# chymaera96/NeuralSampleID

Measured on AMD Instinct MI355X. Metric: audio clips/sec (contrastive step, grafp encoder), higher is better.
Workload: dtype bf16; 1 GPU; B=256 bf16 k=3 hipGraph 2-stream: grafp.yaml GraphEncoder('t') full contrastive step (fwd x2 views + NT-Xent + bwd + clip + Adam), synthetic (64,128) log-mel clip pairs per GPU, random-init weights; global_batch=256, k=3, parallelism=dp1, collectives=none (single process), gemm_arithmetic=bf16 MFMA operands, fp32 accumulate, activation_storage=bf16, views=two HIP streams (parallel graph branches), hipgraph=True

## Files before the change

include/nsid.h:

```cpp
#ifndef NSID_H
#define NSID_H
#include <stddef.h>
#include <stdint.h>

#ifdef __cplusplus
extern "C" {
#endif

#define NSID_OK 0
#define NSID_EINVAL (-1)
#define NSID_ELAUNCH (-2)

#define NSID_ACT_NONE 0
#define NSID_ACT_RELU 1
#define NSID_ACT_LEAKY 2
#define NSID_ACT_ELU 3

#define NSID_ROW_TILE 128

#define NSID_F32 0
#define NSID_BF16 1

#define NSID_GEMM_FP32 0
#define NSID_GEMM_BF16 1
// ... 58 lines not shown
                     float* running_mean, float* running_var, int64_t* num_batches_tracked, float momentum,
                     float eps, float* scale, float* shift, float* mean, float* invstd, void* stream);
int nsid_bn_finalize_deferred(const float* stat, int tiles, int C, int M, const float* gamma, const float* beta, float eps,
                              float* scale, float* shift, float* mean, float* invstd, float* uvar, void* stream);
int nsid_bn_running_update(int n, const int* C, float* const* running_mean, float* const* running_var,
                           int64_t* const* num_batches_tracked, const float* const* mean_a, const float* const* uvar_a,
                           const float* const* mean_b, const float* const* uvar_b, float momentum, void* stream);
int nsid_bn_eval_affine(const float* gamma, const float* beta, const float* running_mean, const float* running_var,
                        float eps, int C, float* scale, float* shift, void* stream);
int nsid_bn_apply(const void* r, const float* scale, const float* shift, int act, const void* residual,
                  void* out, int M, int C, int dtype, void* stream);
int nsid_bn_bwd_reduce(const void* dout, const void* r, int M, int C, const float* scale, const float* shift,
                       const float* mean, const float* invstd, int act, float* partial, int dtype, void* stream);
int nsid_bn_bwd_finalize(const float* partial, int tiles, int C, int M, float* dgamma, float* dbeta, float* coef,
                         void* stream);
int nsid_bn_bwd_finalize_fused(const float* partial, int tiles, int C, int M, float* dgamma, float* dbeta, float* coef,
                               const float* scale, const float* shift, const float* mean, const float* invstd, float* coef4,
                               void* stream);
int nsid_bn_bwd_apply(const void* dout, const void* r, int M, int C, const float* scale, const float* shift,
                      const float* mean, const float* invstd, int act, const float* coef, void* dr, int dtype,
                      void* stream);

int nsid_knn_graph(const void* r, int ldr, const float* scale, const float* shift, int B, int N, int C, int k,
                   int dilation, int32_t* idx, int dtype, void* stream);

int nsid_mr_aggregate_fwd(const void* r, int ldr, const float* scale, const float* shift, const int32_t* idx, int B,
                          int N, int C, int k, void* u, uint8_t* argmax, int dtype, void* stream);
int nsid_mr_aggregate_bwd(const void* du, const int32_t* idx, const uint8_t* argmax, int B, int N, int C, int k,
                          void* dy, int dtype, void* stream);
int nsid_mr_aggregate_bwd_bn(const void* du, const int32_t* idx, const uint8_t* argmax, int B, int N, int C, int k, void* dy,
                             const void* bn_r, int bn_ldr, const float* bn_scale, const float* bn_shift, const float* bn_mean,
                             const float* bn_invstd, int bn_act, float* partial, int dtype, void* stream);

int nsid_batched_index_select_fwd(const float* x, const int32_t* idx, int B, int C, int N, int Nq, int k, float* out,
                                  void* stream);
int nsid_batched_index_select_bwd(const float* dout, const int32_t* idx, int B, int C, int N, int Nq, int k,
                                  float* dx , void* stream);

int nsid_downsample3_fwd(const void* x, int B, int N, int C, const void* wp, int w_dtype, const float* bias, void* out,
                         int Cout, float* stat, int act_dtype, void* stream);
int nsid_downsample3_bwd_weight(const void* dout, const void* x, float* dwp , int B, int N, int C, int Cout,
                                int act_dtype, void* stream);
int nsid_downsample3_bwd_data(const void* dout, const void* wp, const void* w_odd, int w_dtype, void* dx, int B, int N,
                              int C, int Cout, int act_dtype, void* stream);
int nsid_pack_ds_weight_bwd(const float* w, int Cout, int Cin, float* w_odd, void* stream);
int nsid_im2col3_fwd(const void* x, int B, int N, int C, void* col, int dtype, void* stream);
int nsid_im2col3_bwd(const void* dcol, int B, int N, int C, void* dx, int dtype, void* stream);
int nsid_pack_ds_weight(const float* w, int Cout, int Cin, float* wp, void* stream);
int nsid_dsact_fwd(const void* x, int B, int N, int C, const float* in_scale, const float* in_shift, int act_in, const float* w,
                   const float* bias, void* out, int Cout, float* stat, const float* out_scale, const float* out_shift, int act_out,
                   int act_dtype, void* stream);
int nsid_dsact_bwd_weight(const void* dout, const void* x, const float* in_scale, const float* in_shift, int act_in,
                          float* dw , int B, int N, int C, int Cout, int act_dtype, void* stream);
int nsid_dsact_bwd_data(const void* dout, const float* w, void* dx, int B, int N, int C, int Cout, const void* r_prev,
                        const float* scale, const float* shift, const float* mean, const float* invstd, int act, float* partial,
                        int act_dtype, void* stream);
int nsid_dsact_part_rows(int B, int N);
int nsid_ds_prepack(int n, const float* const* w, void* const* wp16, void* const* wb16, float* const* dwp, const int* Cout,
                    const int* Cin, void* stream);
int nsid_unpack_ds_wgrad(const float* dwp, int Cout, int Cin, float* dw , void* stream);

int nsid_peak_patchify_fwd(const float* spec, const float* w, const float* bias, int B, int H, int W, int pb, int pf,
                           int F, void* out, int ldo, float* minmax, int out_dtype, void* stream);
int nsid_peak_patchify_bwd(const float* spec, const float* minmax, const void* out, const void* dout, int ldo,
                           int B, int H, int W, int pb, int pf, int F, float* dw , float* dbias ,
                           int out_dtype, void* stream);
// ... 83 lines not shown
```

neuralsampleid_amd/_lib.py:

```python
import ctypes
import os

import torch

_PKG = os.path.dirname(os.path.abspath(__file__))
LIB_PATH = os.environ.get("NSID_LIB") or os.path.join(_PKG, "libnsid_hip.so")

SIGNATURES = {
    "nsid_set_gemm_precision": "i",
    "nsid_linear_fwd": "pipippiiiiippiipiis",
    "nsid_linear_fwd_res": "pipippipiiiiippiis",
    "nsid_linear_bwd_data": "pipipipiiiiiis",
    "nsid_linear_bwd_data_bn": "pipipipiiiiiipppppips",
    "nsid_linear_bwd_weight": "pipipiiiippiis",
    "nsid_linear_bwd_weight_grouped": "piiis",
    "nsid_colsum_acc": "piiipis",
    "nsid_bn_finalize": "piiipppppffpppps",
    "nsid_bn_finalize_deferred": "piiippfppppps",
    "nsid_bn_running_update": "ippppppppfs",
    "nsid_bn_eval_affine": "ppppfipps",
    "nsid_bn_apply": "pppippiiis",
    "nsid_bn_bwd_reduce": "ppiippppipis",
    "nsid_bn_bwd_finalize": "piiippps",
    "nsid_bn_bwd_apply": "ppiippppippis",
    "nsid_bn_bwd_finalize_fused": "piiipppppppps",
    "nsid_knn_graph": "pippiiiiipis",
    "nsid_mr_aggregate_fwd": "pipppiiiippis",
    "nsid_mr_aggregate_bwd": "pppiiiipis",
    "nsid_im2col3_fwd": "piiipis",
    "nsid_im2col3_bwd": "piiipis",
    "nsid_pack_ds_weight": "piips",
    "nsid_dsact_fwd": "piiippipppipppiis",
    "nsid_dsact_bwd_weight": "ppppipiiiiis",
    "nsid_dsact_bwd_data": "pppiiiipppppipis",
    "nsid_pack_ds_weight_bwd": "piips",
    "nsid_downsample3_fwd": "piiipippipis",
    "nsid_downsample3_bwd_weight": "pppiiiiis",
    "nsid_downsample3_bwd_data": "pppipiiiiis",
    "nsid_unpack_ds_wgrad": "piips",
    "nsid_ds_prepack": "ipppppps",
    "nsid_peak_patchify_fwd": "pppiiiiiipipis",
    "nsid_peak_patchify_bwd": "ppppiiiiiiippis",
    "nsid_peak_patchify_bwd_ws": "ppppiiiiiiipppis",
    "nsid_node_mean_fwd": "piiipis",
    "nsid_node_mean_bwd": "piiipis",
    "nsid_elu_bwd": "pplps",
    "nsid_l2norm_fwd": "piifpps",
    "nsid_l2norm_bwd": "pppiifps",
    "nsid_ntxent_fwd_bwd": "ppiifiipppps",
    "nsid_sumsq_partial": "plps",
    "nsid_adam_step": "pppplpppips",
    "nsid_f32_to_bf16": "ppls",
    "nsid_reflect_pad": "plips",
    "nsid_power_mel_db": "plippiips",
    "nsid_unfold_segments": "piiiiips",
    "nsid_logmel_fft": "pliliippppiplls",
    "nsid_bcn_to_rows": "piiipiis",
    "nsid_rows_to_bcn": "piiiipis",
    "nsid_batched_index_select_fwd": "ppiiiiips",
    "nsid_batched_index_select_bwd": "ppiiiiips",
    "nsid_fill_zero": "pzs",
# ... 137 lines not shown
```

neuralsampleid_amd/csrc/nsid_common.h:

```cpp
#pragma once
#include <hip/hip_runtime.h>
#include <stdint.h>
#include <stdio.h>

#include "../../include/nsid.h"

typedef float f32x2 __attribute__((ext_vector_type(2)));
typedef float f32x4 __attribute__((ext_vector_type(4)));
typedef uint32_t u32x4 __attribute__((ext_vector_type(4)));
typedef __bf16 bf16x4 __attribute__((ext_vector_type(4)));
typedef __bf16 bf16x8 __attribute__((ext_vector_type(8)));

template <typename T> struct Chunk;
template <> struct Chunk<float> {
  static constexpr int N = 4;
  __device__ static __forceinline__ void load(const float* p, float* v) {
    const f32x4 x = *reinterpret_cast<const f32x4*>(p);
#pragma unroll
    for (int e = 0; e < 4; ++e) v[e] = x[e];
  }
  __device__ static __forceinline__ void store(float* p, const float* v) {
    *reinterpret_cast<f32x4*>(p) = f32x4{v[0], v[1], v[2], v[3]};
  }
};
// ... 117 lines not shown
  X(bwd_narrow, -1)                                                                                                           \
  X(g256_min, 512)                                  \
  X(g256_train, 0)                            \
  X(g256_grid, 0)                                           \
  X(wgrad_wide, 1)                                     \
  X(wgrad_rect, 1)                                                                          \
  X(wgrad_wgs_rect, 256)                         \
  X(wgrad_wgs_sq, 1024)                                                                                                       \
  X(wgrad_rect_min, 256)                                                                                                      \
  X(wgrad_sq_min, 256)                                                                                                        \
  X(w3_wgs, 256)                                                                                                              \
  X(w3_min_tiles, 64)                                                                                                         \
  X(knn_strips, 0)                                            \
  X(knn_pair_min, 512)                 \
  X(knn_raw16, 1)               \
  X(knn_raw_wpe, 6)             \
  X(knn_sel_min_n, 128)               \
  X(mr_grid_stride, 0)                              \
  X(mr_split, 0)                                             \
  X(ffn_regs, 3)                \
  X(mr_key_min_k, 8)            \
  X(mr_bwd_sorted_min_k, 3)     \
  X(ffn_waves, 8)                                                \
  X(ffn256, 1)                  \
  X(mrconv_variant, 7)          \
  X(mrconv_pg_wgs, 768)         \
  X(wgg_rows, 4096)             \
  X(wgg_rows_sq, 1024)          \
  X(wgg_rows_gen, 512)          \
  X(bn_fin_tiles, 0)            \
  X(wgg_w3, 1)                  \
  X(wgrad256, 1)                \
  X(wgg_rows256, 4096)          \
  X(ws_gemm, 7)

enum NsidTuneKey {
#define NSID_TUNE_ENUM(name, def) NSID_T_##name,
  NSID_TUNING_TABLE(NSID_TUNE_ENUM)
#undef NSID_TUNE_ENUM
  NSID_T_COUNT
};
extern long g_nsid_tune[NSID_T_COUNT];
static inline long nsid_tune(NsidTuneKey k) { return g_nsid_tune[k]; }

#define NSID_COUNTER_TABLE(X)                                                                  \
  X(gemm_fwd) X(gemm_bwd_data) X(gemm_bwd_weight)              \
  X(gemm_full)                                    \
  X(gemm_ks2)                                                           \
  X(gemm_bwd_split)          \
  X(gemm_split_major)           \
  X(gemm_affine_load)          \
  X(gemm_relu_load)                                                                             \
  X(gemm_bn_sums)              \
  X(gemm_bn_apply_load)     \
  X(gemm256)                                                                   \
  X(ws_fwd) X(ws_bwd_data) X(ws_bwd_bnapply)                    \
  X(wgrad_rect) X(wgrad_square) X(wgrad3) X(wgrad_grouped) X(wgrad_grouped_w3) X(wgrad_grouped_256)                                                 \
  X(bn_bwd_apply) X(bn_bwd_apply_capped)                                                        \
  X(knn2) X(knn2_pair) X(knn2_raw) X(knn_rank) X(knn_sel) X(knn_strips) X(knn_big)                                                  \
  X(mr_fwd_lds) X(mr_fwd_grid) X(mr_fwd_key) X(mr_bwd_sorted)                                                                  \
  X(ffn_fused)                                 \
  X(mrconv_fused)          \
  X(row_sqnorm) X(flat_l2_topk) X(flat_l2_topk_wide) X(seq_scores)    \
  X(clf_node_rows) X(clf_pair_scores)            \
  X(clf_node_rows_n) X(clf_pair_scores_n)        \
  X(clf_mine) X(clf_attn_fwd) X(clf_head_fwd) X(clf_head_bwd) X(clf_attn_bwd) X(clf_seg_reduce)    \
  X(logmel_fft)            \
  X(conv2d_3x3) X(conv2d_1x1) X(ibn_relu) X(stem7_pool) X(gem_pool)

enum NsidCounterKey {
#define NSID_CNT_ENUM(name) NSID_C_##name,
  NSID_COUNTER_TABLE(NSID_CNT_ENUM)
#undef NSID_CNT_ENUM
  NSID_C_COUNT
};
extern long g_nsid_counter[NSID_C_COUNT];
static inline void nsid_count(NsidCounterKey k) { ++g_nsid_counter[k]; }

constexpr int WGG_MAXP = 28;
struct WgProb {
  const void* A[2];
  const void* B[2];
  const float* bsc[2];
  const float* bsh[2];
  float* C;
  int lda, ldb, I, J, R;
  int groups, rchunk;
  int seg_splits, nsplit;
  int tiles, nwg;
  float slope;
  int pad_period, pad_c1;
};
struct WgGroupArgs {
// ... 54 lines not shown
```

neuralsampleid_amd/csrc/wsgemm.hip:

```cpp
#include "nsid_common.h"

namespace {

typedef float f32x16 __attribute__((ext_vector_type(16)));
typedef __attribute__((address_space(3))) void* lds_vptr;
typedef const __attribute__((address_space(1))) void* glb_vptr;
typedef bf16x4 __attribute__((address_space(3)))* lds_bf16x4_ptr;

struct WsArgs {
  const __bf16* x; long ldx;
  const __bf16* w;
  const float* bias;
  const float* in_scale; const float* in_shift; float in_slope;
  __bf16* out; long ldo;
  float* stat; long stat_plane; long stat_ld;
  int M;
};

constexpr int WS_TP = 72;
constexpr int WS_TB = 32 * WS_TP;

template <int CPR>
__device__ __forceinline__ int ws_swz(int j) {
  if constexpr (CPR == 4) return (j >> 2) & 3;
// ... 124 lines not shown
      const bf16x4 v3 = __builtin_amdgcn_ds_read_tr16_b64_v4bf16((lds_bf16x4_ptr)(tr + 4 * WS_TP + 32));
      *reinterpret_cast<bf16x8*>(orow + t * 32) = __builtin_shufflevector(v0, v1, 0, 1, 2, 3, 4, 5, 6, 7);
      *reinterpret_cast<bf16x8*>(orow + 16 * p.ldo + t * 32) = __builtin_shufflevector(v2, v3, 0, 1, 2, 3, 4, 5, 6, 7);
    }

  if constexpr (STAT) {
#pragma unroll
    for (int t = 0; t < GI * NT; ++t) {
      red[((wave * 2 + h) * 2 + 0) * WROWS + t * 32 + j] = ssum[t];
      red[((wave * 2 + h) * 2 + 1) * WROWS + t * 32 + j] = qsum[t];
    }
    __syncthreads();
    for (int c = tid; c < WROWS; c += 256) {
      float s_ = 0.f, q_ = 0.f;
#pragma unroll
      for (int k = 0; k < 8; ++k) { s_ += red[(k * 2 + 0) * WROWS + c]; q_ += red[(k * 2 + 1) * WROWS + c]; }
      const long col = (long)gy * WROWS + c;
      p.stat[(long)tile * p.stat_ld + col] = s_;
      p.stat[p.stat_plane + (long)tile * p.stat_ld + col] = q_;
    }
  }
}

struct WsBwdArgs {
  const __bf16* dy; long ldd;
  const __bf16* w;
  const __bf16* addend; long ldadd;
  __bf16* dx; long ldi;
  const __bf16* bn_r; long bn_ldr;
  const float* bn_scale; const float* bn_shift; const float* bn_mean; const float* bn_invstd; float bn_slope;
  float* bn_partial; long bn_plane; long bn_ld;
  const __bf16* abn_r; const float* abn_coef; long abn_plane; float abn_slope; __bf16* abn_dr; long abn_lddr;
  int M;
};

template <int BPR>
__device__ __forceinline__ int ws_bswz(int row) {
  if constexpr (BPR == 1) return 0;
  else if constexpr (BPR == 2) return (row >> 1) & 1;
  else return row & 3;
}

template <int N, int K, int GI, bool ADD, bool BNR, bool ABN>
__global__ __launch_bounds__(256, (GI * N * K * 2 > 56 * 1024) ? 1 : 2) void ws_bwd_kernel(const WsBwdArgs p) {
  constexpr int KS = N / 16, KT = K / 32;
  constexpr int CPR = K / 8, BPR = K / 32;
  constexpr int WROWS = GI * N, OCH = GI * K;
  constexpr int WBYTES = WROWS * K * 2;
  constexpr int NPIECE = WBYTES / 1024, RPP = 1024 / (2 * K);
  static_assert(N % 16 == 0 && K % 32 == 0 && NPIECE % 4 == 0 && RPP >= 1, "whole fragments, whole pieces per wave");
  constexpr int SIDEB = (ADD || BNR) ? 4 * 2 * 2048 : 0;
  constexpr int REDB = BNR ? 4 * 2 * 2 * OCH * 4 : 0;
  constexpr int COEFB = ABN ? 4 * WROWS * 4 : 0;
  constexpr int LDSB = WBYTES + 4 * WS_TB + SIDEB + REDB + COEFB;
  __shared__ __attribute__((aligned(1024))) char lds[LDSB];
  char* const wimg = lds;
  char* const tb0 = lds + WBYTES;
  char* const side0 = lds + WBYTES + 4 * WS_TB;
  float* const red = reinterpret_cast<float*>(lds + WBYTES + 4 * WS_TB + SIDEB);
  float* const coefs = reinterpret_cast<float*>(lds + WBYTES + 4 * WS_TB + SIDEB + REDB);

  const int tid = threadIdx.x, lane = tid & 63;
  const int wave = __builtin_amdgcn_readfirstlane(tid >> 6);
  const int j = lane & 31, h = lane >> 5;
  const int tile = blockIdx.x, gy = blockIdx.y;
  const long row0 = (long)tile * 128 + wave * 32;

  bf16x8 xf[GI][KS];
  {
    const __bf16* xr = p.dy + (row0 + j) * p.ldd + (long)gy * WROWS + 8 * h;
#pragma unroll
    for (int gi = 0; gi < GI; ++gi)
#pragma unroll
      for (int s = 0; s < KS; ++s) xf[gi][s] = *reinterpret_cast<const bf16x8*>(xr + gi * N + 16 * s);
  }
  bf16x8 rf[ABN ? GI : 1][ABN ? KS : 1];
  if constexpr (ABN) {
    const __bf16* rr = p.abn_r + (row0 + j) * p.ldd + (long)gy * WROWS + 8 * h;
#pragma unroll
    for (int gi = 0; gi < GI; ++gi)
#pragma unroll
      for (int s = 0; s < KS; ++s) rf[gi][s] = *reinterpret_cast<const bf16x8*>(rr + gi * N + 16 * s);
    for (int i = tid; i < WROWS; i += 256) {
#pragma unroll
      for (int v = 0; v < 4; ++v) coefs[v * WROWS + i] = p.abn_coef[v * p.abn_plane + (long)gy * WROWS + i];
    }
  }
  {
    const __bf16* wg = p.w + (long)gy * WROWS * K;
    const int rl = lane / CPR, pc = lane % CPR;
#pragma unroll
    for (int i = 0; i < NPIECE / 4; ++i) {
      const int q = wave * (NPIECE / 4) + i;
      const int row = q * RPP + rl;
      const int lc = (((pc >> 2) ^ ws_bswz<BPR>(row)) << 2) | (pc & 3);
      __builtin_amdgcn_global_load_lds((glb_vptr)(wg + (long)row * K + 8 * lc), (lds_vptr)(wimg + q * 1024), 16, 0, 0);
    }
  }
  const int srow = lane >> 2, scol = 8 * (lane & 3);
  const __bf16* const aptr = ADD ? p.addend + (row0 + srow) * p.ldadd + (long)gy * OCH + scol : nullptr;
  const __bf16* const rptr = BNR ? p.bn_r + (row0 + srow) * p.bn_ldr + (long)gy * OCH + scol : nullptr;
  f32x4 sa[2][2], sr[2][2];
  auto side_load = [&](int t, int par) {
    if constexpr (ADD) {
      sa[par][0] = *reinterpret_cast<const f32x4*>(aptr + t * 32);
      sa[par][1] = *reinterpret_cast<const f32x4*>(aptr + 16 * p.ldadd + t * 32);
    }
    if constexpr (BNR) {
      sr[par][0] = *reinterpret_cast<const f32x4*>(rptr + t * 32);
      sr[par][1] = *reinterpret_cast<const f32x4*>(rptr + 16 * p.bn_ldr + t * 32);
    }
  };
  if constexpr (ADD || BNR) side_load(0, 0);
  wait_vm<0>();
  __syncthreads();

  if constexpr (ABN) {
    const float slope = p.abn_slope;
    const bool masked = slope != 1.f;
    __bf16* const drow = p.abn_dr + (row0 + j) * p.abn_lddr + (long)gy * WROWS + 8 * h;
#pragma unroll
    for (int gi = 0; gi < GI; ++gi)
#pragma unroll
      for (int s = 0; s < KS; ++s) {
        const float* cf = coefs + gi * N + 16 * s + 8 * h;
        const bf16x8 hd = xf[gi][s], hr = rf[gi][s];
        bf16x8 o;
#pragma unroll
        for (int e4 = 0; e4 < 8; e4 += 4) {
          const f32x4 sc = *reinterpret_cast<const f32x4*>(cf + e4), sh = *reinterpret_cast<const f32x4*>(cf + WROWS + e4);
          const f32x4 cp = *reinterpret_cast<const f32x4*>(cf + 2 * WROWS + e4), cq = *reinterpret_cast<const f32x4*>(cf + 3 * WROWS + e4);
#pragma unroll
          for (int e = 0; e < 4; ++e) {
            const float x = (float)hr[e4 + e], d = (float)hd[e4 + e];
            float g = d;
            if (masked) g = (sc[e] * x + sh[e]) > 0.f ? d : d * slope;
            o[e4 + e] = (__bf16)(sc[e] * g + (cp[e] * x + cq[e]));
          }
        }
        xf[gi][s] = o;
        *reinterpret_cast<bf16x8*>(drow + gi * N + 16 * s) = o;
      }
  }

  const int G = lane >> 4, qq = (lane >> 2) & 3, pp = lane & 3;
  const int wq = 8 * h + qq;
  const int wcol = 32 * (G & 1) + 8 * pp;
  char* const tb = tb0 + wave * WS_TB;
  char* const tw = tb + j * WS_TP + 8 * h;
  const char* const tr = tb + (8 * G + qq) * WS_TP + (4 * pp) * 2;
  __bf16* const orow = p.dx + (row0 + (lane & 15)) * p.ldi + (long)gy * OCH + 8 * G;
  char* const simg = side0 + wave * 4096;
  char* const sw_ = simg + lane * 16;
  const char* const sread = simg + (4 * h + qq) * 64 + 32 * (G & 1) + 8 * pp;
  float s0[GI * KT], s1[GI * KT];
#pragma unroll
  for (int t = 0; t < GI * KT; ++t) s0[t] = s1[t] = 0.f;
  const bool bn_unit = p.bn_slope == 1.f;

#pragma unroll
  for (int gi = 0; gi < GI; ++gi)
#pragma unroll
    for (int kt = 0; kt < KT; ++kt) {
      const int t = gi * KT + kt;
      if constexpr (ADD || BNR) {
        if (t + 1 < GI * KT) side_load(t + 1, (t + 1) & 1);
      }
      f32x16 acc;
#pragma unroll
      for (int r = 0; r < 16; ++r) acc[r] = 0.f;
#pragma unroll
      for (int s = 0; s < KS; ++s) {
        const int ra = gi * N + 16 * s + wq, rb = ra + 4;
        const bf16x4 w0 = __builtin_amdgcn_ds_read_tr16_b64_v4bf16(
            (lds_bf16x4_ptr)(wimg + ra * (2 * K) + ((kt ^ ws_bswz<BPR>(ra)) << 6) + wcol));
        const bf16x4 w1 = __builtin_amdgcn_ds_read_tr16_b64_v4bf16(
            (lds_bf16x4_ptr)(wimg + rb * (2 * K) + ((kt ^ ws_bswz<BPR>(rb)) << 6) + wcol));
        acc = __builtin_amdgcn_mfma_f32_32x32x16_bf16(xf[gi][s], __builtin_shufflevector(w0, w1, 0, 1, 2, 3, 4, 5, 6, 7), acc, 0, 0, 0);
      }
      if constexpr (ADD) {
        *reinterpret_cast<f32x4*>(sw_) = sa[t & 1][0];
        *reinterpret_cast<f32x4*>(sw_ + 1024) = sa[t & 1][1];
#pragma unroll
        for (int g = 0; g < 4; ++g) {
          const bf16x4 a4 = __builtin_amdgcn_ds_read_tr16_b64_v4bf16((lds_bf16x4_ptr)(sread + 512 * g));
#pragma unroll
          for (int e = 0; e < 4; ++e) acc[4 * g + e] += (float)a4[e];
        }
      }
      bf16x4 o4[4];
#pragma unroll
      for (int g = 0; g < 4; ++g) {
        o4[g] = __builtin_convertvector((f32x4{acc[4 * g], acc[4 * g + 1], acc[4 * g + 2], acc[4 * g + 3]}), bf16x4);
        *reinterpret_cast<bf16x4*>(tw + 16 * g) = o4[g];
      }
      if constexpr (BNR) {
        *reinterpret_cast<f32x4*>(sw_ + 2048) = sr[t & 1][0];
        *reinterpret_cast<f32x4*>(sw_ + 2048 + 1024) = sr[t & 1][1];
        const long ch = (long)gy * OCH + t * 32 + j;
        const float bsc = p.bn_scale[ch], bsh = p.bn_shift[ch], bmu = p.bn_mean[ch], bis = p.bn_invstd[ch];
        float a0 = 0.f, a1 = 0.f;
#pragma unroll
        for (int g = 0; g < 4; ++g) {
          const bf16x4 r4 = __builtin_amdgcn_ds_read_tr16_b64_v4bf16((lds_bf16x4_ptr)(sread + 2048 + 512 * g));
#pragma unroll
          for (int e = 0; e < 4; ++e) {
            const float dyv = (float)o4[g][e], xx = (float)r4[e];
            float gg = dyv;
            if (!bn_unit) gg = (bsc * xx + bsh) > 0.f ? dyv : dyv * p.bn_slope;
            a0 += gg;
            a1 += gg * ((xx - bmu) * bis);
          }
        }
        s0[t] = a0; s1[t] = a1;
      }
      const bf16x4 v0 = __builtin_amdgcn_ds_read_tr16_b64_v4bf16((lds_bf16x4_ptr)(tr));
      const bf16x4 v1 = __builtin_amdgcn_ds_read_tr16_b64_v4bf16((lds_bf16x4_ptr)(tr + 4 * WS_TP));
      const bf16x4 v2 = __builtin_amdgcn_ds_read_tr16_b64_v4bf16((lds_bf16x4_ptr)(tr + 32));
      const bf16x4 v3 = __builtin_amdgcn_ds_read_tr16_b64_v4bf16((lds_bf16x4_ptr)(tr + 4 * WS_TP + 32));
      *reinterpret_cast<bf16x8*>(orow + t * 32) = __builtin_shufflevector(v0, v1, 0, 1, 2, 3, 4, 5, 6, 7);
      *reinterpret_cast<bf16x8*>(orow + 16 * p.ldi + t * 32) = __builtin_shufflevector(v2, v3, 0, 1, 2, 3, 4, 5, 6, 7);
    }

  if constexpr (BNR) {
#pragma unroll
    for (int t = 0; t < GI * KT; ++t) {
      red[((wave * 2 + h) * 2 + 0) * OCH + t * 32 + j] = s0[t];
      red[((wave * 2 + h) * 2 + 1) * OCH + t * 32 + j] = s1[t];
    }
    __syncthreads();
    for (int c = tid; c < OCH; c += 256) {
      float a0 = 0.f, a1 = 0.f;
#pragma unroll
      for (int k = 0; k < 8; ++k) { a0 += red[(k * 2 + 0) * OCH + c]; a1 += red[(k * 2 + 1) * OCH + c]; }
      const long col = (long)gy * OCH + c;
      p.bn_partial[(long)tile * p.bn_ld + col] = a0;
      p.bn_partial[p.bn_plane + (long)tile * p.bn_ld + col] = a1;
    }
  }
}

template <int N, int K, int GI>
int ws_bwd_launch_t(const WsBwdArgs& p, int gy, hipStream_t s) {
  const dim3 grid(p.M / 128, gy), block(256);
  const bool add = p.addend != nullptr, bnr = p.bn_r != nullptr;
#define WS_BWD_GO(ABN_)                                                                                   \
  do {                                                                                                    \
    if (add) {                                                                                            \
      if (bnr) NSID_LAUNCH((ws_bwd_kernel<N, K, GI, true, true, ABN_>), grid, block, 0, s, p);             \
      else NSID_LAUNCH((ws_bwd_kernel<N, K, GI, true, false, ABN_>), grid, block, 0, s, p);                \
    } else {                                                                                              \
      if (bnr) NSID_LAUNCH((ws_bwd_kernel<N, K, GI, false, true, ABN_>), grid, block, 0, s, p);            \
      else NSID_LAUNCH((ws_bwd_kernel<N, K, GI, false, false, ABN_>), grid, block, 0, s, p);               \
    }                                                                                                     \
  } while (0)
  if (p.abn_r != nullptr) WS_BWD_GO(true);
  else WS_BWD_GO(false);
#undef WS_BWD_GO
  return nsid_launch_status();
}

template <int K, int NOUT, int GI>
int ws_launch(const WsArgs& p, int gy, bool aff, bool stat, hipStream_t s) {
  const dim3 grid(p.M / 128, gy), block(256);
  if (aff) {
    if constexpr (GI > 1) return 1;
    else {
      if (stat) NSID_LAUNCH((ws_fwd_kernel<K, NOUT, GI, true, true>), grid, block, 0, s, p);
      else NSID_LAUNCH((ws_fwd_kernel<K, NOUT, GI, true, false>), grid, block, 0, s, p);
    }
  } else {
    if (stat) NSID_LAUNCH((ws_fwd_kernel<K, NOUT, GI, false, true>), grid, block, 0, s, p);
    else NSID_LAUNCH((ws_fwd_kernel<K, NOUT, GI, false, false>), grid, block, 0, s, p);
  }
  return nsid_launch_status();
}

}

__attribute__((visibility("hidden")))
int nsid_ws_fwd_launch(const void* x, int ldx, const void* w, const float* bias, void* out, int ldo, int M, int Nout, int K,
                       int groups, const float* in_scale, const float* in_shift, float in_slope, float* stat, long stat_plane,
                       long stat_ld, hipStream_t stream) {
  if (M % 128 != 0 || ldx % 8 != 0 || ldo % 8 != 0 || ldx < groups * K || ldo < groups * Nout) return 1;
  if (!nsid_aligned16(x) || !nsid_aligned16(w) || !nsid_aligned16(out)) return 1;
  if ((in_scale != nullptr) != (in_shift != nullptr)) return 1;
  if (in_scale && (!nsid_aligned16(in_scale) || !nsid_aligned16(in_shift))) return 1;
  WsArgs p{};
  p.x = static_cast<const __bf16*>(x); p.ldx = ldx;
  p.w = static_cast<const __bf16*>(w);
  p.bias = bias;
// ... 25 lines not shown
                            const void* abn_r, const float* abn_coef, long abn_plane, float abn_slope, void* abn_dr, long abn_lddr,
                            hipStream_t stream) {
  if (abn_r && (!abn_coef || !abn_dr || ldd != groups * Nout || abn_lddr % 8 != 0 || !nsid_aligned16(abn_r) || !nsid_aligned16(abn_dr) ||
                !nsid_aligned16(abn_coef) || abn_plane % 4 != 0)) return 1;
  if (M % 128 != 0 || ldd % 8 != 0 || ldi % 8 != 0 || ldd < groups * Nout || ldi < groups * K) return 1;
  if (!nsid_aligned16(dout) || !nsid_aligned16(w) || !nsid_aligned16(din)) return 1;
  if (addend && (ldadd % 8 != 0 || ldadd < groups * K || !nsid_aligned16(addend))) return 1;
  if (bn_r && (bn_ldr % 8 != 0 || !nsid_aligned16(bn_r) || !bn_scale || !bn_shift || !bn_mean || !bn_invstd || !bn_partial)) return 1;
  WsBwdArgs p{};
  p.dy = static_cast<const __bf16*>(dout); p.ldd = ldd;
  p.w = static_cast<const __bf16*>(w);
  p.addend = static_cast<const __bf16*>(addend); p.ldadd = ldadd;
  p.dx = static_cast<__bf16*>(din); p.ldi = ldi;
  p.bn_r = static_cast<const __bf16*>(bn_r); p.bn_ldr = bn_ldr;
  p.bn_scale = bn_scale; p.bn_shift = bn_shift; p.bn_mean = bn_mean; p.bn_invstd = bn_invstd; p.bn_slope = bn_slope;
  p.bn_partial = bn_partial; p.bn_plane = bn_plane; p.bn_ld = bn_ld;
  p.abn_r = static_cast<const __bf16*>(abn_r); p.abn_coef = abn_coef; p.abn_plane = abn_plane; p.abn_slope = abn_slope;
  p.abn_dr = static_cast<__bf16*>(abn_dr); p.abn_lddr = abn_lddr;
  p.M = M;
#define WS_CASE(N_, K_, G_, GI_)                                                   \
  if (Nout == N_ && K == K_ && groups == G_) return ws_bwd_launch_t<N_, K_, GI_>(p, G_ / GI_, stream)
  WS_CASE(64, 64, 1, 1);
  WS_CASE(32, 32, 4, 4);
  WS_CASE(64, 128, 1, 1);
  WS_CASE(256, 64, 1, 1);
  WS_CASE(64, 256, 1, 1);
  WS_CASE(128, 128, 1, 1);
  WS_CASE(64, 64, 4, 4);
  WS_CASE(128, 256, 1, 1);
  WS_CASE(128, 128, 4, 1);
#undef WS_CASE
  return 1;
}
```

neuralsampleid_amd/functional.py:

```python
from typing import Dict, List, Optional

import torch

from . import ops
from .ops import ACT_ELU, ACT_LEAKY, ACT_NONE, ACT_RELU, BNAffine

Tensor = torch.Tensor


class KnnTape:

    def __init__(self, replay: Optional[List[Tensor]] = None, cyclic: bool = False, patch=None):
        self.replay = list(replay) if replay is not None else None
        self.recorded: List[Tensor] = []
        self.pos = 0
        self.cyclic = cyclic
        self.patch = list(patch) if patch is not None else None
        self.patched: List[Tensor] = []


TAPE: Optional[KnnTape] = None

EXACT_BIAS_GRAD = False

# ... 296 lines not shown
    if fold_eval(training, S) and a1 is not None and a1.identity:
        gg, gb, grm, grv, _, _ = _bn(P, S, pre + "1.")
        wgf, bgf = ops.folded_conv_bn(ops.w2d(P[pre + "0.weight"]), P[pre + "0.bias"], gg, gb, grm, grv)
        r2, a2 = ops.mrconv_fused_fwd(r1, idx, B, N, C, wgf, bgf), None
    if r2 is None:
        u, amax = ops.mr_aggregate_fwd(r1, idx, B, N, C, a1, want_argmax=S is not None)
        r2, a2 = conv_bn(u, M, C // 2, C // 2, P[pre + "0.weight"], P[pre + "0.bias"], _bn(P, S, pre + "1."), training,
                         groups=4, folded_act=ACT_RELU)
    if fold_eval(training, S):
        return conv_bn(r2, M, 2 * C, C, P["fc2.0.weight"], P["fc2.0.bias"], _bn(P, S, "fc2.1."), training,
                       in_aff=a2, act_in=ACT_RELU, residual=x0)[0]
    r3, a3 = conv_bn(r2, M, 2 * C, C, P["fc2.0.weight"], P["fc2.0.bias"], _bn(P, S, "fc2.1."), training,
                     in_aff=a2, act_in=ACT_RELU)
    x1 = ops.bn_apply(r3, a3, ACT_NONE, residual=x0)
    if S is not None:
        S.update(x0=x0, r1=r1, a1=a1, idx=idx, amax=amax, u=u, r2=r2, a2=a2, r3=r3, a3=a3, B=B, N=N)
        if CHAIN is not None:
            CHAIN.consume(S)
            CHAIN.produce(S, r3, a3, ACT_NONE)
    return x1


def grapher_backward(dx1: Tensor, P, S, G) -> Tensor:
    x0, r1, a1, idx, amax, u, r2, a2, r3, a3 = (S[k_] for k_ in ("x0", "r1", "a1", "idx", "amax", "u", "r2", "a2",
                                                                  "r3", "a3"))
    B, N = S["B"], S["N"]
    M, C = x0.shape
    pre = "graph_conv.gconv.nn."
    dr3, dv, part2 = ops.bn_backward_linear_bwd_data(dx1, r3, a3, ACT_NONE, G["fc2.1.weight"], G["fc2.1.bias"], _link_partial(S),
                                                     ops.w2d(P["fc2.0.weight"]), M, C, 2 * C, 1, bn=(r2, a2, ACT_RELU),
                                                     site=ops.SITE_FC2, inplace=False)
    _bias_grad_before_bn(dr3, G["fc2.0.bias"])
    _wgrad(dr3, r2, ops.w2d(G["fc2.0.weight"]), M, C, 2 * C, 1, a2.scale, a2.shift, ACT_RELU)
    dr2, du, _ = ops.bn_backward_linear_bwd_data(dv, r2, a2, ACT_RELU, G[pre + "1.weight"], G[pre + "1.bias"], part2,
                                                 ops.w2d(P[pre + "0.weight"]), M, C // 2, C // 2, 4, site=ops.SITE_GCONV)
    _bias_grad_before_bn(dr2, G[pre + "0.bias"])
    _wgrad(dr2, u, ops.w2d(G[pre + "0.weight"]), M, C // 2, C // 2, 4)
    dy, part1 = ops.mr_aggregate_bwd(du, idx, amax, B, N, C, bn=(r1, a1, ACT_NONE))
    dr1, dx0, part = ops.bn_backward_linear_bwd_data(dy, r1, a1, ACT_NONE, G["fc1.1.weight"], G["fc1.1.bias"], part1,
                                                     ops.w2d(P["fc1.0.weight"]), M, C, C, 1, addend=dx1, bn=_link_in(S) or False,
                                                     site=ops.SITE_FC1)
    _bias_grad_before_bn(dr1, G["fc1.0.bias"])
    _wgrad(dr1, x0, ops.w2d(G["fc1.0.weight"]), M, C, C)
    _store_partial(S, part)
    return dx0


def ffn_forward(x1: Tensor, P, S: Optional[dict], training: bool) -> Tensor:
    M, C = x1.shape
    H = P["fc1.0.weight"].shape[0]
    if fold_eval(training, S) and C in (64, 128, 256) and H == 4 * C and M % (256 if C == 256 else 128) == 0:
        g1, be1, rm1, rv1, _, _ = _bn(P, S, "fc1.1.")
        g2, be2, rm2, rv2, _, _ = _bn(P, S, "fc2.1.")
        w1f, b1f = ops.folded_conv_bn(ops.w2d(P["fc1.0.weight"]), None, g1, be1, rm1, rv1)
        w2f, b2f = ops.folded_conv_bn(ops.w2d(P["fc2.0.weight"]), None, g2, be2, rm2, rv2)
        out = ops.ffn_fused_fwd(x1, w1f, b1f, w2f, b2f, M, C, H)
        if out is not None:
            return out
    r4, a4 = conv_bn(x1, M, C, H, P["fc1.0.weight"], None, _bn(P, S, "fc1.1."), training, folded_act=ACT_RELU)
    if fold_eval(training, S):
        return conv_bn(r4, M, H, C, P["fc2.0.weight"], None, _bn(P, S, "fc2.1."), training, in_aff=a4, act_in=ACT_RELU,
                       residual=x1)[0]
    r5, a5 = conv_bn(r4, M, H, C, P["fc2.0.weight"], None, _bn(P, S, "fc2.1."), training, in_aff=a4, act_in=ACT_RELU)
    x2 = ops.bn_apply(r5, a5, ACT_NONE, residual=x1)
    if S is not None:
        S.update(x1=x1, r4=r4, a4=a4, r5=r5, a5=a5)
        if CHAIN is not None:
            CHAIN.consume(S)
            CHAIN.produce(S, r5, a5, ACT_NONE)
    return x2

# ... 295 lines not shown
```

neuralsampleid_amd/ops.py:

```python
import os
from typing import Optional, Tuple

import torch

from ._lib import call, get_tuning, launch_counters, lib, reset_tuning, set_tuning

ACT_NONE, ACT_RELU, ACT_LEAKY, ACT_ELU = 0, 1, 2, 3
ROW_TILE = 128
BN_MOMENTUM = 0.1
BN_EPS = 1e-5


class KernelProfile:

    def __init__(self):
        self.records = []
        self.bracket_ms = self._empty_bracket_ms()

    @staticmethod
    def plug(ms: float = 120.0) -> None:
        torch.cuda._sleep(int(ms * 1e-3 * 2.0e9))

    @staticmethod
    def _empty_bracket_ms(n: int = 64) -> float:
# ... 688 lines not shown
def mr_bwd_sums_fused(du, N, C, k) -> bool:
    kmin = get_tuning("mr_bwd_sorted_min_k")
    return bool(FUSE_MR_BWD_SUMS and du.dtype == torch.bfloat16 and kmin > 0 and k >= kmin and N * C == 16384 and C & (C - 1) == 0
                and 64 <= C <= 512)


FUSE_MR_BWD_SUMS = True


def mr_aggregate_bwd(du, idx, amax, B, N, C, bn=None):
    dt = _act(du)
    k = idx.shape[-1]
    dy = torch.empty((B * N, C), device=du.device, dtype=du.dtype)
    nbytes = float(B) * N * (3 * C * du.element_size() + k * 4 + C)
    if bn is not None and mr_bwd_sums_fused(du, N, C, k):
        r, aff, act = bn
        _chk(aff.scale, aff.shift, aff.mean, aff.invstd)
        partial = torch.empty((2, B, C), device=du.device, dtype=torch.float32)
        rc = [0]

        def launch():
            rc[0] = lib.nsid_mr_aggregate_bwd_bn(_p(du), _p(idx), _p(amax), B, N, C, k, _p(dy), _p(r), r.shape[-1], _p(aff.scale),
                                                 _p(aff.shift), _p(aff.mean), _p(aff.invstd), act, _p(partial), dt, _stream())
        _timed("mr_bwd_sorted_kernel +bn_sums", 0.0, nbytes + float(B) * N * C * r.element_size(), launch, (B * N, C, 2 * C, 1))
        if rc[0] == 0:
            return dy, partial
        if PROFILE is not None:
            PROFILE.records.pop()
    c0 = _cnt("mr_bwd_sorted")
    _timed(lambda: "mr_bwd_sorted_kernel" if _cnt("mr_bwd_sorted") > c0 else "mr_bwd_kernel", 0.0, nbytes, lambda: call(
        "nsid_mr_aggregate_bwd", _p(du), _p(idx), _p(amax), B, N, C, k, _p(dy), dt, _stream()),
        (B * N, C, 2 * C, 1))
    return (dy, None) if bn is not None else dy


def ds_out_nodes(N: int) -> int:
    return (N - 1) // 2 + 1


def im2col3_fwd(x, B, N, C) -> torch.Tensor:
    dt = _act(x)
    col = torch.empty((B * ds_out_nodes(N), 3 * C), device=x.device, dtype=x.dtype)
    call("nsid_im2col3_fwd", _p(x), B, N, C, _p(col), dt, _stream())
    return col


def im2col3_bwd(dcol, B, N, C) -> torch.Tensor:
    dt = _act(dcol)
    dx = torch.empty((B * N, C), device=dcol.device, dtype=dcol.dtype)
    call("nsid_im2col3_bwd", _p(dcol), B, N, C, _p(dx), dt, _stream())
    return dx


class DsPrep:

    def __init__(self):
        self.entries = {}

    MAX_LAYERS = 8

    def purge(self) -> None:
        for ptr in [k for k, e in self.entries.items() if e["wref"]() is None or e["wref"]().data_ptr() != k]:
            del self.entries[ptr]

    def register(self, w) -> None:
        import weakref
# ... 711 lines not shown
```

Baseline: 35930 clips/s.

## Fuse grouped-conv backward data with max-relative aggregation backward and BN sums

Adds a templated AGG variant of the ws_bwd_kernel that keeps the grouped-conv input gradient in LDS instead of writing it out. Inside the same tile it builds a per-node CSR of neighbour sources and scatters the max-relative aggregation backward using the argmax indices. It then accumulates the downstream BN backward partial sums before writing. This removes the separate mr_aggregate_bwd launch and the du round trip through global memory. In exchange it adds LDS pressure, per-tile atomics and serial neighbour loops, and it only works when each 128-row tile holds whole clips (N divides 128), with a fallback path otherwise.

After: 36250 clips/s, median of 6. Within noise of the previous version (+0.9%).

```diff
diff --git a/include/nsid.h b/include/nsid.h
--- a/include/nsid.h
+++ b/include/nsid.h
@@ -114,6 +114,13 @@
                              const void* bn_r, int bn_ldr, const float* bn_scale, const float* bn_shift, const float* bn_mean,
                              const float* bn_invstd, int bn_act, float* partial, int dtype, void* stream);
 
+int nsid_gconv_bwd_aggr(const void* dy, const void* r, const float* coef4, int act, void* dr, const void* w, int w_dtype,
+                        const void* addend, int ldadd, void* din, int ldi, int M, int Nout, int K, int groups, int act_dtype,
+                        const void* bn_r, const float* bn_scale, const float* bn_shift, const float* bn_mean, const float* bn_invstd,
+                        int bn_act, float* bn_partial, const int32_t* idx, const uint8_t* argmax, int B, int N, int k, void* agg_dy,
+                        const void* agg_r, int agg_ldr, const float* agg_scale, const float* agg_shift, const float* agg_mean,
+                        const float* agg_invstd, int agg_act, float* agg_partial, void* stream);
+
 int nsid_batched_index_select_fwd(const float* x, const int32_t* idx, int B, int C, int N, int Nq, int k, float* out,
                                   void* stream);
 int nsid_batched_index_select_bwd(const float* dout, const int32_t* idx, int B, int C, int N, int Nq, int k,
diff --git a/neuralsampleid_amd/_lib.py b/neuralsampleid_amd/_lib.py
--- a/neuralsampleid_amd/_lib.py
+++ b/neuralsampleid_amd/_lib.py
@@ -27,6 +27,7 @@
     "nsid_knn_graph": "pippiiiiipis",
     "nsid_mr_aggregate_fwd": "pipppiiiippis",
     "nsid_mr_aggregate_bwd": "pppiiiipis",
+    "nsid_gconv_bwd_aggr": "pppippipipiiiiiipppppip" + "ppiii" + "ppippppip" + "s",
     "nsid_im2col3_fwd": "piiipis",
     "nsid_im2col3_bwd": "piiipis",
     "nsid_pack_ds_weight": "piips",
diff --git a/neuralsampleid_amd/csrc/nsid_common.h b/neuralsampleid_amd/csrc/nsid_common.h
--- a/neuralsampleid_amd/csrc/nsid_common.h
+++ b/neuralsampleid_amd/csrc/nsid_common.h
@@ -173,7 +173,9 @@
   X(wgg_w3, 1)                  \
   X(wgrad256, 1)                \
   X(wgg_rows256, 4096)          \
-  X(ws_gemm, 7)
+  X(ws_gemm, 7)                 \
+  X(gconv_bwd_aggr, 1)          \
+  X(gconv_bwd_aggr_max_k, 8)
 
 enum NsidTuneKey {
 #define NSID_TUNE_ENUM(name, def) NSID_T_##name,
@@ -199,7 +201,7 @@
   X(wgrad_rect) X(wgrad_square) X(wgrad3) X(wgrad_grouped) X(wgrad_grouped_w3) X(wgrad_grouped_256)                                                 \
   X(bn_bwd_apply) X(bn_bwd_apply_capped)                                                        \
   X(knn2) X(knn2_pair) X(knn2_raw) X(knn_rank) X(knn_sel) X(knn_strips) X(knn_big)                                                  \
-  X(mr_fwd_lds) X(mr_fwd_grid) X(mr_fwd_key) X(mr_bwd_sorted)                                                                  \
+  X(mr_fwd_lds) X(mr_fwd_grid) X(mr_fwd_key) X(mr_bwd_sorted) X(gconv_bwd_aggr)                                                             \
   X(ffn_fused)                                 \
   X(mrconv_fused)          \
   X(row_sqnorm) X(flat_l2_topk) X(flat_l2_topk_wide) X(seq_scores)    \
diff --git a/neuralsampleid_amd/csrc/wsgemm.hip b/neuralsampleid_amd/csrc/wsgemm.hip
--- a/neuralsampleid_amd/csrc/wsgemm.hip
+++ b/neuralsampleid_amd/csrc/wsgemm.hip
@@ -180,7 +180,13 @@
   float* bn_partial; long bn_plane; long bn_ld;
   const __bf16* abn_r; const float* abn_coef; long abn_plane; float abn_slope; __bf16* abn_dr; long abn_lddr;
   int M;
+  const int32_t* ag_idx; const uint8_t* ag_amax; __bf16* ag_dy; int ag_N; int ag_k; int ag_C;
+  const __bf16* ag_r; long ag_ldr;
+  const float* ag_scale; const float* ag_shift; const float* ag_mean; const float* ag_invstd; float ag_slope;
+  float* ag_partial; long ag_plane;
 };
+
+constexpr int WS_AG_KMAX = 32;
 
 template <int BPR>
 __device__ __forceinline__ int ws_bswz(int row) {
@@ -189,7 +195,7 @@
   else return row & 3;
 }
 
-template <int N, int K, int GI, bool ADD, bool BNR, bool ABN>
+template <int N, int K, int GI, bool ADD, bool BNR, bool ABN, bool AGG = false>
 __global__ __launch_bounds__(256, (GI * N * K * 2 > 56 * 1024) ? 1 : 2) void ws_bwd_kernel(const WsBwdArgs p) {
   constexpr int KS = N / 16, KT = K / 32;
   constexpr int CPR = K / 8, BPR = K / 32;
@@ -200,8 +206,18 @@
   constexpr int SIDEB = (ADD || BNR) ? 4 * 2 * 2048 : 0;
   constexpr int REDB = BNR ? 4 * 2 * 2 * OCH * 4 : 0;
   constexpr int COEFB = ABN ? 4 * WROWS * 4 : 0;
-  constexpr int LDSB = WBYTES + 4 * WS_TB + SIDEB + REDB + COEFB;
+  static_assert(!AGG || (ABN && !ADD && !BNR), "the aggregation form exists for the grouped-conv site only");
+  constexpr int CH = OCH / 2;
+  constexpr int AG_OS = 2 * CH + 8, AG_AS = CH + 4;
+  constexpr int AG0 = WBYTES + 4 * WS_TB + SIDEB + REDB + COEFB;
+  constexpr int AGB = AGG ? 128 * AG_AS + 128 * 4 + 132 * 4 + 128 * WS_AG_KMAX * 2 : 0;
+  constexpr int LDSB = AG0 + AGB;
+  static_assert(!AGG || (128 * AG_OS <= WBYTES + 4 * WS_TB && LDSB <= 80 * 1024 && AG0 % 16 == 0), "two workgroups per CU");
   __shared__ __attribute__((aligned(1024))) char lds[LDSB];
+  char* const ag_am = lds + AG0;
+  int* const ag_cnt = reinterpret_cast<int*>(lds + AG0 + 128 * AG_AS);
+  int* const ag_start = ag_cnt + 128;
+  uint16_t* const ag_src = reinterpret_cast<uint16_t*>(ag_start + 132);
   char* const wimg = lds;
   char* const tb0 = lds + WBYTES;
   char* const side0 = lds + WBYTES + 4 * WS_TB;
@@ -243,6 +259,40 @@
       const int row = q * RPP + rl;
       const int lc = (((pc >> 2) ^ ws_bswz<BPR>(row)) << 2) | (pc & 3);
       __builtin_amdgcn_global_load_lds((glb_vptr)(wg + (long)row * K + 8 * lc), (lds_vptr)(wimg + q * 1024), 16, 0, 0);
+    }
+  }
+  if constexpr (AGG) {
+    const int k = p.ag_k, E = 128 * k, cn = p.ag_N;
+    const int32_t* const nbb = p.ag_idx + (long)tile * 128 * k;
+    if (tid < 128) ag_cnt[tid] = 0;
+    const uint8_t* const amb = p.ag_amax + (long)tile * 128 * p.ag_C + gy * CH;
+    for (int q = tid; q < 128 * (CH / 16); q += 256) {
+      const int row = q / (CH / 16), c16 = q % (CH / 16);
+      const u32x4 a = *reinterpret_cast<const u32x4*>(amb + (long)row * p.ag_C + 16 * c16);
+      uint32_t* const d = reinterpret_cast<uint32_t*>(ag_am + row * AG_AS + 16 * c16);
+      d[0] = a[0]; d[1] = a[1]; d[2] = a[2]; d[3] = a[3];
+    }
+    __syncthreads();
+    for (int e = tid; e < E; e += 256) {
+      const int m = e / k;
+      atomicAdd(&ag_cnt[(m / cn) * cn + min(max(nbb[e], 0), cn - 1)], 1);
+    }
+    __syncthreads();
+    if (tid < 64) {
+      const int c0 = ag_cnt[2 * tid], c1 = ag_cnt[2 * tid + 1];
+      int inc = c0 + c1;
+#pragma unroll
+      for (int o2 = 1; o2 < 64; o2 <<= 1) { const int v = __shfl_up(inc, o2, 64); if (tid >= o2) inc += v; }
+      const int run = inc - c0 - c1;
+      ag_start[2 * tid] = run; ag_cnt[2 * tid] = run;
+      ag_start[2 * tid + 1] = run + c0; ag_cnt[2 * tid + 1] = run + c0;
+      if (tid == 63) ag_start[128] = inc;
+    }
+    __syncthreads();
+    for (int e = tid; e < E; e += 256) {
+      const int m = e / k;
+      const int pos = atomicAdd(&ag_cnt[(m / cn) * cn + min(max(nbb[e], 0), cn - 1)], 1);
+      ag_src[pos] = (uint16_t)((m << 8) | (e - m * k));
     }
   }
   const int srow = lane >> 2, scol = 8 * (lane & 3);
@@ -304,6 +354,7 @@
   float s0[GI * KT], s1[GI * KT];
 #pragma unroll
   for (int t = 0; t < GI * KT; ++t) s0[t] = s1[t] = 0.f;
+  u32x4 du8[AGG ? 2 : 1][AGG ? GI * KT : 1];
   const bool bn_unit = p.bn_slope == 1.f;
 
 #pragma unroll
@@ -366,9 +417,95 @@
       const bf16x4 v1 = __builtin_amdgcn_ds_read_tr16_b64_v4bf16((lds_bf16x4_ptr)(tr + 4 * WS_TP));
       const bf16x4 v2 = __builtin_amdgcn_ds_read_tr16_b64_v4bf16((lds_bf16x4_ptr)(tr + 32));
       const bf16x4 v3 = __builtin_amdgcn_ds_read_tr16_b64_v4bf16((lds_bf16x4_ptr)(tr + 4 * WS_TP + 32));
-      *reinterpret_cast<bf16x8*>(orow + t * 32) = __builtin_shufflevector(v0, v1, 0, 1, 2, 3, 4, 5, 6, 7);
-      *reinterpret_cast<bf16x8*>(orow + 16 * p.ldi + t * 32) = __builtin_shufflevector(v2, v3, 0, 1, 2, 3, 4, 5, 6, 7);
-    }
+      if constexpr (AGG) {
+        du8[0][t] = __builtin_bit_cast(u32x4, __builtin_shufflevector(v0, v1, 0, 1, 2, 3, 4, 5, 6, 7));
+        du8[1][t] = __builtin_bit_cast(u32x4, __builtin_shufflevector(v2, v3, 0, 1, 2, 3, 4, 5, 6, 7));
+      } else {
+        *reinterpret_cast<bf16x8*>(orow + t * 32) = __builtin_shufflevector(v0, v1, 0, 1, 2, 3, 4, 5, 6, 7);
+        *reinterpret_cast<bf16x8*>(orow + 16 * p.ldi + t * 32) = __builtin_shufflevector(v2, v3, 0, 1, 2, 3, 4, 5, 6, 7);
+      }
+    }
+
+  if constexpr (AGG) {
+    constexpr int T = GI * KT;
+    char* const odd = lds;
+    const int rl = wave * 32 + (lane & 15);
+    __syncthreads();
+    float own[2][T][4];
+#pragma unroll
+    for (int rr = 0; rr < 2; ++rr)
+#pragma unroll
+      for (int t = 0; t < T; ++t) {
+        const u32x4 w4 = du8[rr][t];
+        *reinterpret_cast<uint2*>(odd + (rl + 16 * rr) * AG_OS + 2 * (16 * t + 4 * G)) =
+            uint2{(w4[0] >> 16) | (w4[1] & 0xffff0000u), (w4[2] >> 16) | (w4[3] & 0xffff0000u)};
+#pragma unroll
+        for (int e = 0; e < 4; ++e) own[rr][t][e] = __uint_as_float(w4[e] << 16) - __uint_as_float(w4[e] & 0xffff0000u);
+      }
+    __syncthreads();
+#pragma unroll
+    for (int rr = 0; rr < 2; ++rr) {
+      const int p1 = ag_start[rl + 16 * rr + 1];
+      for (int q = ag_start[rl + 16 * rr]; q < p1; ++q) {
+        const uint32_t s2 = ag_src[q];
+        const uint32_t m = s2 >> 8, jj = s2 & 255u;
+        const char* const ob = odd + m * AG_OS + 8 * G;
+        const char* const ab = ag_am + m * AG_AS + 4 * G;
+#pragma unroll
+        for (int t = 0; t < T; ++t) {
+          const uint2 o = *reinterpret_cast<const uint2*>(ob + 32 * t);
+          const uint32_t a = *reinterpret_cast<const uint32_t*>(ab + 16 * t);
+          own[rr][t][0] += (a & 255u) == jj ? __uint_as_float(o.x << 16) : 0.f;
+          own[rr][t][1] += ((a >> 8) & 255u) == jj ? __uint_as_float(o.x & 0xffff0000u) : 0.f;
+          own[rr][t][2] += ((a >> 16) & 255u) == jj ? __uint_as_float(o.y << 16) : 0.f;
+          own[rr][t][3] += (a >> 24) == jj ? __uint_as_float(o.y & 0xffff0000u) : 0.f;
+        }
+      }
+    }
+    __syncthreads();
+    float* const red = reinterpret_cast<float*>(lds);
+    const bool masked = p.ag_slope != 1.f;
+    const long grow = (long)tile * 128 + rl;
+#pragma unroll
+    for (int t = 0; t < T; ++t) {
+      const int cl = 16 * t + 4 * G;
+      const long ch = (long)gy * CH + cl;
+      const f32x4 bmu = *reinterpret_cast<const f32x4*>(p.ag_mean + ch), bis = *reinterpret_cast<const f32x4*>(p.ag_invstd + ch);
+      f32x4 bsc = {1.f, 1.f, 1.f, 1.f}, bsh = {0.f, 0.f, 0.f, 0.f};
+      if (masked) { bsc = *reinterpret_cast<const f32x4*>(p.ag_scale + ch); bsh = *reinterpret_cast<const f32x4*>(p.ag_shift + ch); }
+      float a0[4] = {0.f, 0.f, 0.f, 0.f}, a1[4] = {0.f, 0.f, 0.f, 0.f};
+#pragma unroll
+      for (int rr = 0; rr < 2; ++rr) {
+        const bf16x4 o4 = __builtin_convertvector((f32x4{own[rr][t][0], own[rr][t][1], own[rr][t][2], own[rr][t][3]}), bf16x4);
+        *reinterpret_cast<bf16x4*>(p.ag_dy + (grow + 16 * rr) * p.ag_C + ch) = o4;
+        const bf16x4 x4 = *reinterpret_cast<const bf16x4*>(p.ag_r + (grow + 16 * rr) * p.ag_ldr + ch);
+#pragma unroll
+        for (int e = 0; e < 4; ++e) {
+          const float dyv = (float)o4[e], xx = (float)x4[e];
+          float gg = dyv;
+          if (masked) gg = (bsc[e] * xx + bsh[e]) > 0.f ? dyv : dyv * p.ag_slope;
+          a0[e] += gg;
+          a1[e] += gg * ((xx - bmu[e]) * bis[e]);
+        }
+      }
+#pragma unroll
+      for (int o2 = 1; o2 < 16; o2 <<= 1)
+#pragma unroll
+        for (int e = 0; e < 4; ++e) { a0[e] += __shfl_xor(a0[e], o2, 64); a1[e] += __shfl_xor(a1[e], o2, 64); }
+      if ((lane & 15) == 0) {
+        *reinterpret_cast<f32x4*>(red + (wave * 2 + 0) * CH + cl) = f32x4{a0[0], a0[1], a0[2], a0[3]};
+        *reinterpret_cast<f32x4*>(red + (wave * 2 + 1) * CH + cl) = f32x4{a1[0], a1[1], a1[2], a1[3]};
+      }
+    }
+    __syncthreads();
+    const int cpt = 128 / p.ag_N, wpc = 4 / cpt;
+    for (int i = tid; i < cpt * 2 * CH; i += 256) {
+      const int clip = i / (2 * CH), which = (i / CH) & 1, c = i % CH;
+      float a = 0.f;
+      for (int w2 = 0; w2 < wpc; ++w2) a += red[((clip * wpc + w2) * 2 + which) * CH + c];
+      p.ag_partial[which * p.ag_plane + ((long)tile * cpt + clip) * p.ag_C + gy * CH + c] = a;
+    }
+  }
 
   if constexpr (BNR) {
 #pragma unroll
@@ -405,6 +542,12 @@
   if (p.abn_r != nullptr) WS_BWD_GO(true);
   else WS_BWD_GO(false);
 #undef WS_BWD_GO
+  return nsid_launch_status();
+}
+
+template <int N, int K, int GI>
+int ws_bwd_aggr_launch_t(const WsBwdArgs& p, int gy, hipStream_t s) {
+  NSID_LAUNCH((ws_bwd_kernel<N, K, GI, false, false, true, true>), dim3(p.M / 128, gy), dim3(256), 0, s, p);
   return nsid_launch_status();
 }
 
@@ -496,3 +639,44 @@
 #undef WS_CASE
   return 1;
 }
+
+extern "C" int nsid_gconv_bwd_aggr(const void* dy, const void* r, const float* coef4, int act, void* dr, const void* w, int w_dtype,
+                                   const void* addend, int ldadd, void* din, int ldi, int M, int Nout, int K, int groups, int act_dtype,
+                                   const void* bn_r, const float* bn_scale, const float* bn_shift, const float* bn_mean,
+                                   const float* bn_invstd, int bn_act, float* bn_partial, const int32_t* idx, const uint8_t* argmax, int B,
+                                   int N, int k, void* agg_dy, const void* agg_r, int agg_ldr, const float* agg_scale,
+                                   const float* agg_shift, const float* agg_mean, const float* agg_invstd, int agg_act, float* agg_partial,
+                                   void* stream) {
+  (void)ldadd; (void)din; (void)ldi; (void)bn_scale; (void)bn_shift; (void)bn_mean; (void)bn_invstd; (void)bn_act; (void)bn_partial;
+  NSID_REQUIRE(dy && r && coef4 && dr && w && idx && argmax && agg_dy && agg_r && agg_scale && agg_shift && agg_mean && agg_invstd &&
+               agg_partial && M > 0 && Nout > 0 && K > 0 && groups > 0 && B > 0 && N > 0 && k > 0 && k <= 255);
+  NSID_REQUIRE(NSID_DTYPE_OK(act_dtype) && NSID_DTYPE_OK(w_dtype) && (long)B * N == (long)M && dr != dy && dr != r);
+  NSID_REQUIRE(act == NSID_ACT_NONE || act == NSID_ACT_RELU || act == NSID_ACT_LEAKY);
+  NSID_REQUIRE(agg_act == NSID_ACT_NONE || agg_act == NSID_ACT_RELU || agg_act == NSID_ACT_LEAKY);
+  if (nsid_tune(NSID_T_gconv_bwd_aggr) == 0 || act_dtype != NSID_BF16 || w_dtype != NSID_BF16 || addend != nullptr || bn_r != nullptr)
+    return 1;
+  if (N > 128 || 128 % N != 0 || M % 128 != 0 || k > WS_AG_KMAX || k > nsid_tune(NSID_T_gconv_bwd_aggr_max_k) || groups != 4 || Nout != K)
+    return 1;
+  if (!((K == 64 && N == 128) || (K == 128 && N == 64))) return 1;
+  const int C = groups * K / 2;
+  NSID_REQUIRE(agg_ldr % 8 == 0 && agg_ldr >= C && nsid_aligned16(dy) && nsid_aligned16(r) && nsid_aligned16(coef4) && nsid_aligned16(dr) &&
+               nsid_aligned16(w) && nsid_aligned16(argmax) && nsid_aligned16(agg_dy) && nsid_aligned16(agg_r) && nsid_aligned16(agg_scale) &&
+               nsid_aligned16(agg_shift) && nsid_aligned16(agg_mean) && nsid_aligned16(agg_invstd));
+  auto slope_of = [](int a) { return a == NSID_ACT_RELU ? 0.f : (a == NSID_ACT_LEAKY ? 0.2f : 1.f); };
+  WsBwdArgs p{};
+  p.dy = static_cast<const __bf16*>(dy); p.ldd = (long)groups * Nout;
+  p.w = static_cast<const __bf16*>(w);
+  p.ldi = (long)groups * K;
+  p.abn_r = static_cast<const __bf16*>(r); p.abn_coef = coef4; p.abn_plane = (long)groups * Nout; p.abn_slope = slope_of(act);
+  p.abn_dr = static_cast<__bf16*>(dr); p.abn_lddr = (long)groups * Nout;
+  p.bn_slope = 1.f;
+  p.M = M;
+  p.ag_idx = idx; p.ag_amax = argmax; p.ag_dy = static_cast<__bf16*>(agg_dy); p.ag_N = N; p.ag_k = k; p.ag_C = C;
+  p.ag_r = static_cast<const __bf16*>(agg_r); p.ag_ldr = agg_ldr;
+  p.ag_scale = agg_scale; p.ag_shift = agg_shift; p.ag_mean = agg_mean; p.ag_invstd = agg_invstd; p.ag_slope = slope_of(agg_act);
+  p.ag_partial = agg_partial; p.ag_plane = (long)B * C;
+  nsid_count(NSID_C_gconv_bwd_aggr);
+  hipStream_t s = static_cast<hipStream_t>(stream);
+  if (K == 64) return ws_bwd_aggr_launch_t<64, 64, 4>(p, 1, s);
+  return ws_bwd_aggr_launch_t<128, 128, 1>(p, 4, s);
+}
diff --git a/neuralsampleid_amd/functional.py b/neuralsampleid_amd/functional.py
--- a/neuralsampleid_amd/functional.py
+++ b/neuralsampleid_amd/functional.py
@@ -352,11 +352,17 @@
                                                      site=ops.SITE_FC2, inplace=False)
     _bias_grad_before_bn(dr3, G["fc2.0.bias"])
     _wgrad(dr3, r2, ops.w2d(G["fc2.0.weight"]), M, C, 2 * C, 1, a2.scale, a2.shift, ACT_RELU)
-    dr2, du, _ = ops.bn_backward_linear_bwd_data(dv, r2, a2, ACT_RELU, G[pre + "1.weight"], G[pre + "1.bias"], part2,
-                                                 ops.w2d(P[pre + "0.weight"]), M, C // 2, C // 2, 4, site=ops.SITE_GCONV)
+    fused = ops.gconv_bwd_aggregate(dv, r2, a2, ACT_RELU, G[pre + "1.weight"], G[pre + "1.bias"], part2, ops.w2d(P[pre + "0.weight"]),
+                                    M, C // 2, C // 2, 4, idx, amax, B, N, C, bn=(r1, a1, ACT_NONE))
+    if fused is not None:
+        dr2, dy, part1 = fused
+    else:
+        dr2, du, _ = ops.bn_backward_linear_bwd_data(dv, r2, a2, ACT_RELU, G[pre + "1.weight"], G[pre + "1.bias"], part2,
+                                                     ops.w2d(P[pre + "0.weight"]), M, C // 2, C // 2, 4, site=ops.SITE_GCONV)
     _bias_grad_before_bn(dr2, G[pre + "0.bias"])
     _wgrad(dr2, u, ops.w2d(G[pre + "0.weight"]), M, C // 2, C // 2, 4)
-    dy, part1 = ops.mr_aggregate_bwd(du, idx, amax, B, N, C, bn=(r1, a1, ACT_NONE))
+    if fused is None:
+        dy, part1 = ops.mr_aggregate_bwd(du, idx, amax, B, N, C, bn=(r1, a1, ACT_NONE))
     dr1, dx0, part = ops.bn_backward_linear_bwd_data(dy, r1, a1, ACT_NONE, G["fc1.1.weight"], G["fc1.1.bias"], part1,
                                                      ops.w2d(P["fc1.0.weight"]), M, C, C, 1, addend=dx1, bn=_link_in(S) or False,
                                                      site=ops.SITE_FC1)
diff --git a/neuralsampleid_amd/ops.py b/neuralsampleid_amd/ops.py
--- a/neuralsampleid_amd/ops.py
+++ b/neuralsampleid_amd/ops.py
@@ -744,6 +744,55 @@
         "nsid_mr_aggregate_bwd", _p(du), _p(idx), _p(amax), B, N, C, k, _p(dy), dt, _stream()),
         (B * N, C, 2 * C, 1))
     return (dy, None) if bn is not None else dy
+
+
+FUSE_GCONV_BWD_AGGR = 1
+
+
+def gconv_bwd_aggregate(dv, r2, a2: "BNAffine", act, dgamma, dbeta, partial, w, M, Nout, K, groups, idx, amax, B, N, C, bn):
+    k = idx.shape[-1]
+    if not (FUSE_GCONV_BWD_AGGR and partial is not None and dv.dtype == torch.bfloat16 and r2.dtype == torch.bfloat16 and
+            M == B * N and M % 128 == 0 and groups == 4 and Nout == K and (K, N) in ((64, 128), (128, 64)) and 2 * C == groups * K and
+            k <= min(32, get_tuning("gconv_bwd_aggr_max_k")) and tuple(r2.shape) == (M, groups * Nout) and tuple(dv.shape) == (M, groups * Nout) and
+            get_tuning("gconv_bwd_aggr") != 0):
+        return None
+    dt = _act(dv, r2)
+    wop, wdt = _weight(w, dt, K)
+    r1, a1, act1 = bn
+    if wdt != BF16 or r1.dtype != torch.bfloat16 or tuple(r1.shape) != (M, C):
+        return None
+    _chk(a1.scale, a1.shift, a1.mean, a1.invstd)
+    s = _stream()
+    ptiles = partial.shape[1]
+    CC = groups * Nout
+    coef = torch.empty((6, CC), device=r2.device, dtype=torch.float32)
+    if not (DIAG_SKIP_FINALIZE & 2):
+        _tk("bn_bwd_finalize_kernel", 8.0 * ptiles * CC + 40.0 * CC, lambda: call(
+            "nsid_bn_bwd_finalize_fused", _p(partial), ptiles, CC, M, _p(dgamma), _p(dbeta), _p(coef), _p(a2.scale), _p(a2.shift),
+            _p(a2.mean), _p(a2.invstd), _p(coef[2]), s), (M, CC, 0, 1))
+    dr = torch.empty_like(dv)
+    dy = torch.empty((M, C), device=dv.device, dtype=dv.dtype)
+    part1 = torch.empty((2, B, C), device=dv.device, dtype=torch.float32)
+    esz = dv.element_size()
+    nbytes = groups * (3 * esz * M * Nout + float(wop.element_size()) * Nout * K) + float(M) * (2 * esz * C + C + 4 * k)
+    rc = [0]
+
+    def launch():
+        rc[0] = lib.nsid_gconv_bwd_aggr(
+            _p(dv), _p(r2), _p(coef[2]), act, _p(dr), _p(wop), wdt, None, 0, None, groups * K, M, Nout, K, groups, dt, None, None, None,
+            None, None, ACT_NONE, None, _p(idx), _p(amax), B, N, k, _p(dy), _p(r1), r1.shape[-1], _p(a1.scale), _p(a1.shift), _p(a1.mean),
+            _p(a1.invstd), act1, _p(part1), s)
+    _timed("ws_bwd_kernel +bn_apply_load", 2.0 * M * Nout * K * groups, nbytes, launch, (M, Nout, K, groups))
+    if rc[0] == 0:
+        return dr, dy, part1
+    if rc[0] != 1:
+        raise RuntimeError(f"nsid_gconv_bwd_aggr failed: {rc[0]}")
+    if PROFILE is not None:
+        PROFILE.records.pop()
+    call("nsid_bn_bwd_apply", _p(dv), _p(r2), M, CC, _p(a2.scale), _p(a2.shift), _p(a2.mean), _p(a2.invstd), act, _p(coef), _p(dr), dt, s)
+    du = linear_bwd_data(dr, w, M, Nout, K, groups, bn=False)[0]
+    dy, part1 = mr_aggregate_bwd(du, idx, amax, B, N, C, bn=bn)
+    return dr, dy, part1
 
 
 def ds_out_nodes(N: int) -> int:
```
